# ajzhai/PEANUT

Measured on AMD Instinct MI355X. Metric: maps/sec for 480x480x(4+N_cat) prediction fwd, batch 32, higher is better.
Workload: dtype f32; 1 GPU; 480x480, 14-channel (4+10) partial maps -> 6-class prediction forward (PSPNet R50-V1c-D8), batch 32 per GPU, seeded random-init weights; survey_config=2, global_batch=32, parallelism=dp1 (map shards, no data-path collective)

## Files before the change

include/peanut_hip.h:

```cpp
#ifndef PEANUT_HIP_H_
#define PEANUT_HIP_H_

#include <stddef.h>
#include <stdint.h>

#ifdef __cplusplus
extern "C" {
#endif

#define PEANUT_OK 0
#define PEANUT_EINVAL (-2)
#define PEANUT_EHIP (-3)
#define PEANUT_EWEIGHTS (-4)
#define PEANUT_ERANGE (-5)

const char* peanut_last_error(void);
const char* peanut_last_conv_kernel(void);
int peanut_abi_version(void);
const char* peanut_build_arch(void);
const char* peanut_source_hash(void);
int peanut_debug_weight_pieces(const float* values, int n, int precision, unsigned short* pieces, float* pack_scale);
int peanut_debug_wino_weights(const float* w_oihw, int cout, int cin, int tile, float* out);
long long peanut_debug_deferred_splitk_count(void);
int peanut_debug_lds_canary(int workgroups, int lds_bytes, int rounds, int* mismatches, void* stream);
int peanut_debug_pkfma_canary(int workgroups, int rounds, int* mismatches, void* stream);

int peanut_set_default_option(const char* key, long long value);
int peanut_get_default_option(const char* key, long long* value);
const char* peanut_option_list(void);


typedef struct peanut_pred_cfg {
  int in_channels;
  int num_classes;
  int strides[4];
  int dilations[4];
  int contract_dilation;
  int pool_scales[8];
  int n_pool_scales;
  int head_channels;
  int align_corners;
  float bn_eps;
  int precision;
  int fold_ppm;
  int conv_algo;
} peanut_pred_cfg;

#define PEANUT_ALGO_AUTO 0
#define PEANUT_ALGO_DIRECT 1

#define PEANUT_PREC_FP32 0
#define PEANUT_PREC_BF16X3 1
#define PEANUT_PREC_FP16X3 2
#define PEANUT_PREC_BF16X6 3

typedef struct peanut_tensor {
// ... 191 lines not shown
```

peanut_amd/_lib.py:

```python
from __future__ import annotations

import ctypes as C
import os
import threading

import torch

from . import build as _build

_LOCK = threading.Lock()
_LIB = None
ABI_VERSION = 17


class PeanutHipError(RuntimeError):
    pass


class PeanutRangeError(PeanutHipError, FloatingPointError):
    """PEANUT_ERANGE: precision fp16x3 and a value left fp16's exponent range (include/peanut_hip.h)."""


class PredCfgC(C.Structure):
    _fields_ = [
        ("in_channels", C.c_int), ("num_classes", C.c_int),
        ("strides", C.c_int * 4), ("dilations", C.c_int * 4), ("contract_dilation", C.c_int),
        ("pool_scales", C.c_int * 8), ("n_pool_scales", C.c_int),
        ("head_channels", C.c_int), ("align_corners", C.c_int), ("bn_eps", C.c_float),
        ("precision", C.c_int), ("fold_ppm", C.c_int), ("conv_algo", C.c_int),
    ]


class MapCfgC(C.Structure):
    _fields_ = [
        ("frame_height", C.c_int), ("frame_width", C.c_int), ("map_resolution", C.c_int),
        ("map_size_cm", C.c_int), ("global_downscaling", C.c_int), ("vision_range", C.c_int),
        ("hfov", C.c_double), ("du_scale", C.c_int),
        ("cat_pred_threshold", C.c_double), ("exp_pred_threshold", C.c_double),
        ("map_pred_threshold", C.c_double), ("num_sem_categories", C.c_int), ("camera_height", C.c_double),
    ]


class RcnnCfgC(C.Structure):
    _fields_ = [
        ("depth", C.c_int), ("stem_out", C.c_int), ("res2_out", C.c_int), ("stride_in_1x1", C.c_int),
        ("fpn_out", C.c_int), ("num_anchors", C.c_int), ("min_size", C.c_int), ("max_size", C.c_int),
        ("size_divisibility", C.c_int), ("pixel_mean", C.c_float * 3), ("pixel_std", C.c_float * 3),
        ("bn_eps", C.c_float), ("precision", C.c_int), ("conv_algo", C.c_int),
        ("anchor_sizes", C.c_float * 5), ("aspect_ratios", C.c_float * 8),
        ("rpn_pre_nms_topk", C.c_int), ("rpn_post_nms_topk", C.c_int), ("rpn_nms_thresh", C.c_float),
        ("rpn_bbox_weights", C.c_float * 4), ("num_classes", C.c_int), ("box_pooler_resolution", C.c_int),
        ("mask_pooler_resolution", C.c_int), ("fc_dim", C.c_int), ("mask_conv_dim", C.c_int), ("num_mask_convs", C.c_int),
        ("roi_bbox_weights", C.c_float * 4), ("score_thresh_test", C.c_float), ("nms_thresh_test", C.c_float),
        ("detections_per_image", C.c_int), ("mask_threshold", C.c_float),
    ]


class TensorC(C.Structure):
    _fields_ = [("name", C.c_char_p), ("data", C.c_void_p), ("ndim", C.c_int), ("shape", C.c_int64 * 4)]


_P = C.c_void_p
SIGNATURES = {
    "peanut_last_error": (C.c_char_p, []),
    "peanut_last_conv_kernel": (C.c_char_p, []),
    "peanut_abi_version": (C.c_int, []),
    "peanut_build_arch": (C.c_char_p, []),
    "peanut_source_hash": (C.c_char_p, []),
    "peanut_debug_weight_pieces": (C.c_int, [C.c_void_p, C.c_int, C.c_int, C.c_void_p, C.POINTER(C.c_float)]),
    "peanut_debug_wino_weights": (C.c_int, [C.c_void_p, C.c_int, C.c_int, C.c_int, C.c_void_p]),
    "peanut_debug_deferred_splitk_count": (C.c_longlong, []),
    "peanut_debug_lds_canary": (C.c_int, [C.c_int, C.c_int, C.c_int, C.c_void_p, C.c_void_p]),
    "peanut_debug_pkfma_canary": (C.c_int, [C.c_int, C.c_int, C.c_void_p, C.c_void_p]),
    "peanut_pred_create": (C.c_int, [C.POINTER(_P), C.POINTER(PredCfgC), C.POINTER(TensorC), C.c_int]),
    "peanut_pred_destroy": (None, [_P]),
    "peanut_pred_forward": (C.c_int, [_P, _P, _P, C.c_int, C.c_int, C.c_int, C.c_int, _P]),
    "peanut_pred_workspace_bytes": (C.c_size_t, [_P, C.c_int, C.c_int, C.c_int]),
    "peanut_pred_flops_per_map": (C.c_double, [_P, C.c_int, C.c_int]),
    "peanut_pred_debug_keep": (C.c_int, [_P, C.c_int]),
    "peanut_pred_debug_tensor": (C.c_int, [_P, C.c_char_p, C.POINTER(_P), C.POINTER(C.c_int * 4)]),
    "peanut_pred_debug_read": (C.c_int, [_P, C.c_char_p, _P, C.c_size_t, C.POINTER(C.c_int * 4), _P]),
    "peanut_pred_probe_enable": (C.c_int, [_P, C.c_int]),
    "peanut_pred_use_graph": (C.c_int, [_P, C.c_int]),
    "peanut_map_use_graph": (C.c_int, [_P, C.c_int]),
    "peanut_map_mark_agent": (C.c_int, [_P, C.c_int, C.c_int, C.c_int, C.c_int, C.c_int, C.c_int, _P, C.c_int, C.c_int, _P, _P]),
    "peanut_pred_probe_collect": (C.c_int, [_P, C.c_int, C.POINTER(C.c_char_p), C.POINTER(C.c_char_p),
                                            C.POINTER(C.c_double), C.POINTER(C.c_double), C.POINTER(C.c_double),
                                            C.POINTER(C.c_int)]),
    "peanut_map_create": (C.c_int, [C.POINTER(_P), C.POINTER(MapCfgC)]),
    "peanut_map_destroy": (None, [_P]),
    "peanut_map_dims": (C.c_int, [_P, C.POINTER(C.c_int * 4)]),
    "peanut_map_forward": (C.c_int, [_P, _P, _P, _P, _P, _P, _P, _P]),
    "peanut_map_reserve": (C.c_int, [_P, C.c_int]),
    "peanut_map_forward_batch": (C.c_int, [_P, C.c_int, _P, _P, C.POINTER(_P), _P, _P, C.POINTER(_P), _P]),
    "peanut_map_mark_agent_batch": (C.c_int, [C.c_int, C.POINTER(_P), C.c_int, C.c_int, C.POINTER(C.c_int), _P, C.c_int,
                                              C.POINTER(C.c_int), C.POINTER(C.c_int), _P]),
    "peanut_map_debug_launches": (C.c_int, [_P]),
    "peanut_preprocess_obs_batch": (C.c_int, [_P, _P, _P, C.c_int, C.c_int, C.c_int, C.c_int, C.c_int, C.c_double, C.c_double, _P, _P]),
# ... 161 lines not shown
```

peanut_amd/csrc/common.h:

```cpp
#pragma once
#include <hip/hip_runtime.h>
#include <stdint.h>
#include <string>

namespace peanut {

void set_error(const std::string& msg);
int fail(int code, const std::string& msg);
void note_kernel(const char* family);
const char* noted_kernel();

#define PEANUT_HIP_CHECK(expr)                                                            \
  do {                                                                                    \
    hipError_t _e = (expr);                                                               \
    if (_e != hipSuccess)                                                                 \
      return ::peanut::fail(-3, std::string(#expr) + ": " + hipGetErrorString(_e));       \
  } while (0)

struct ConvDesc {
  int cin;
  int cout;
  int kh, kw, stride, pad, dil;
  int relu;
  int bn_tile;
// ... 60 lines not shown
  };
  return at(y0, x0) * wy * wx + at(y0, x0 + 1) * wy * lx + at(y0 + 1, x0) * ly * wx + at(y0 + 1, x0 + 1) * ly * lx;
}

inline int conv_out_dim(int n, int k, int s, int p, int d) { return (n + 2 * p - d * (k - 1) - 1) / s + 1; }

void conv_pick_tiles(int cin_pad, int cout, int* bn_tile, int* bk, bool pointwise = false);
size_t conv_packed_floats(int cin_pad, int cout, int kh, int kw, int bn_tile);
void pack_conv_weights(const float* w_oihw, int cout, int cin_real, int cin_pad, int kh, int kw,
                       int bn_tile, int bk, float* out);
int launch_conv(const ConvDesc& d, const ConvArgs& a, hipStream_t stream);
bool conv_pw_enabled();
bool conv_pw_uses_256(int cout, long long M, int mt_per_group, int bn_tile, int cin);
int conv_pw_256_min_k();
bool conv_pw_uses_256w(int cout, long long M, int mt_per_group, int bn_tile, int cin, int flush_ktiles);
bool conv_pw_narrow_tiles(int cin, int cout, long long M, int bn_tile, int mt_per_group);
bool conv_pw_uses_256p(int cout, long long M, int mt_per_group, int bn_tile, int cin, int flush_ktiles, long long in_pixels = 0);
struct ConvKParams;
bool gemm_skinny_takes(const ConvKParams& p, int bn_tile, size_t ws_floats);
int launch_gemm_skinny(const ConvKParams& p, float* ws, size_t ws_floats, hipStream_t stream);
bool conv_pw_uses_256wp(int cout, long long M, int stride, int mt_per_group, int bn_tile, int c1, int c2, int flush_ktiles);
bool conv_pw_uses_ares(int cin, int cout, long long M, int stride, bool two_source, int flush_ktiles, int bn_tile);

bool conv_patch_eligible(const ConvDesc& d, const ConvArgs& a);
const char* conv_patch_kernel_name(const ConvDesc& d, bool nchw);
bool conv_patch_nchw_eligible(const ConvDesc& d, int B, int Ho, int Wo, int creal);
int launch_conv_patch_nchw(const ConvDesc& d, const float* x_nchw, int creal, float* y, int B, int H, int W, int Ho, int Wo, hipStream_t stream);

void wino_geometry(int B, int H, int W, int dil, int* th, int* tw, long long* n_tiles, long long* m_pad, int gran = 128, int m = 4);
void wino_transform_weights(const float* w_oihw, int cout, int cin, float* out, int m = 4);
int launch_wino_input(const float* x, float* V, int B, int H, int W, int C, int dil, hipStream_t s, int gran = 128, int m = 4, long long m_pad_total = 0,
                      const DeferredSplit* df = nullptr);
bool wino_input_accepts_deferred(int B, int H, int W, int C, int dil, int gran, int m);
long long wino_deferred_count();
int launch_wino_output(const float* Mb, const float* scale, const float* shift, const float* res, float* y,
                       int B, int H, int W, int C, int dil, int relu, hipStream_t s, int gran = 128, int m = 4, long long m_pad_total = 0);

bool gemm_rs_uses_256(int cout, long long M, int mt_per_group, int bn_tile, int cin);
const char* gemm_rs_kernel_name(int cout, long long M, int mt_per_group, int bn_tile, int cin, int planes);
size_t sx_packed_bytes(int cin_pad, int cout, int bn_tile, int planes);
void pack_weights_sx(const float* w, int cout, int cin_real, int cin_pad, int bn_tile, int planes, float wscale, void* out);
float sx_pack_scale(const float* w, size_t n, int planes);
size_t sx_conv_packed_bytes(int cin_pad, int cout, int kh, int kw, int bn_tile, int planes);
void pack_weights_sx_conv(const float* w_oihw, int cout, int cin_real, int cin_pad, int kh, int kw, int bn_tile, int planes,
                          float wscale, void* out);

int launch_nchw_to_nhwc_pad(const float* x, float* y, int B, int C, int H, int W, int Cpad, hipStream_t s);
int launch_maxpool3x3s2(const float* x, float* y, int B, int H, int W, int C, int Ho, int Wo, hipStream_t s);
int launch_ppm_pool(const float* x, float* out, int B, int H, int W, int C, const int* scales, int nscales,
                    hipStream_t s, int scale_rows = 0);
size_t ppm_pool_scratch_floats(int B, int H, int C, const int* scales, int nscales);
int launch_ppm_pool2(const float* x, float* scratch, float* out, int B, int H, int W, int C, const int* scales,
                     int nscales, hipStream_t s, int scale_rows = 0);
int launch_ppm_upsample_concat(const float* table, float* out, int B, int H, int W, int Cp, const int* scales,
                               int nscales, int align_corners, hipStream_t s);
int launch_ppm_conv_term(const float* Q, float* R, int B, int H, int W, int C, const int* scales, int nscales,
                         int align_corners, hipStream_t s, int scale_rows = 0);
int launch_upsample_logits(const float* lo, float* out, int B, int h, int w, int K, int H, int W,
                           int align_corners, int sigmoid, hipStream_t s);

}
```

peanut_amd/csrc/options.h:

```cpp
#pragma once
#include <stdlib.h>
#include <string.h>

#include <string>

namespace peanut {

enum OptionId {
  OPT_PW_GLDS, OPT_PW256_MINK, OPT_PW256_MINTILES, OPT_PW256_PHASE, OPT_PW256_SKIP_PAD, OPT_PW256W_MINK, OPT_PW256W_MINTILES, OPT_PW256P_MINK, OPT_PW256P_MINTILES, OPT_PW256P_FLUSH, OPT_PW256P_ORDER, OPT_PW256P_STREAMK, OPT_PW256WP_MINK, OPT_PW256WP_MINTILES, OPT_PW256WP_NPRE, OPT_PW256WP_STAGGER, OPT_PW_ARES, OPT_PW_SKINNY,
  OPT_PW_ARES_MINUNITS, OPT_PATCH_MINTILES, OPT_STEM_NCHW, OPT_BN64_MAXK, OPT_PW_BN64_MAXK, OPT_PW64_MAXTILES, OPT_FP32_BK, OPT_NCHUNK, OPT_RES_PREFETCH, OPT_SPLIT_MODEL,
  OPT_RS_CONV, OPT_RS_BN64_MAXK, OPT_RS256_MINK, OPT_RS256_MINTILES, OPT_RS64_MAXK, OPT_RS64_MAXTILES,
  OPT_WINO_M, OPT_WINO_HEAD_M, OPT_WINO6_MAXDIL, OPT_WINO5_MINDIL, OPT_WINO_FLUSH_CH, OPT_WINO_MIN_CIN, OPT_WINO_NARROW_MINPIX, OPT_WINO_SMALL_MAXWG, OPT_DEFER_SPLITK,
  OPT_PPM_OVERLAP, OPT_PPM_GROUPED, OPT_PPM_TERM_ROWS, OPT_PPM_GROUP_ROWS, OPT_RCNN_WINO_M, OPT_RCNN_STEM_S2D, OPT_RCNN_RPN_FUSED, OPT_RCNN_FPN_OVERLAP, OPT_RCNN_RANK_SORT, OPT_RCNN_TOPK_SLICE, OPT_RCNN_NMS_LEVELS, OPT_FMM_LOCAL32, OPT_FMM_MAX_PASSES, OPT_FMM_BLOCKED, OPT_FMM_INNER,
  OPT_COUNT
};

struct OptionInfo {
  const char* key;
  long long def;
  bool upload_time;
  const char* help;
};

inline const OptionInfo* option_table() {
  static const OptionInfo t[OPT_COUNT] = {
      {"pw_glds", 1, false, "fp32 1x1 convs / grouped GEMMs on the LDS-DMA kernels of conv_pw.hip (0: conv_igemm)"},
      {"pw256_mink", 1024, false, "fewest input channels for the 256 x 128 three-stage kernel"},
      {"pw256_mintiles", 256, false, "fewest 256 x 128 tiles for that kernel"},
      {"pw256_phase", 1, false, "the two waves of a SIMD request their LDS-DMA pieces half an iteration apart"},
      {"pw256_skip_pad", 1, false, "256 x 128 kernel, grouped GEMMs: waves whose rows are all group padding issue no MFMAs (0: compute the zero rows)"},
      {"pw256w_mink", 768, false, "fewest input channels for the 256 x 256 two-stage kernel (0: off)"},
      {"pw256w_mintiles", 1536, false, "fewest 256 x 256 tiles for that kernel"},
      {"pw256p_mink", 512, false, "fewest input channels for the persistent 256 x 128 kernel (conv_pw256p.hip; 0: off)"},
      {"pw256p_mintiles", 512, false, "fewest 256 x 128 tiles for that kernel"},
      {"pw256p_flush", 512, false, "most input channels of a Winograd position GEMM (two-level accumulation) that runs on the persistent kernel (0: none)"},
      {"pw256p_order", 1, false, "persistent 256 x 128 kernel: 1 = the workgroups of an XCD walk its run of tiles side by side (neighbours share operand panels in L2), 0 = one contiguous run per workgroup"},
      {"pw256p_streamk", 1, false, "persistent 256 x 128 kernel: the tail tiles' k-tiles as one stream in equal runs per workgroup (0: every tail tile cut into the same number of parts)"},
      {"pw256wp_mink", 512, false, "fewest input channels for the persistent 256 x 256 kernel (conv_pw256wp.hip; 0: off)"},
      {"pw256wp_mintiles", 768, false, "fewest 256 x 256 tiles for that kernel"},
      {"pw256wp_npre", 0, false, "persistent 256 x 256 kernel: accumulator blocks per in-place epilogue group (2 or 4; 0 = two with a residual, four without)"},
      {"pw256wp_stagger", 0, false, "persistent 256 x 256 kernel: spread of the workgroups' start times in sleeps of ~3.4 us (their tile boundaries -- 512 KiB of epilogue traffic per CU -- then fall at different times)"},
      {"pw_ares", 1, false, "K = 128 / 256 pointwise layers on the persistent A-resident kernel (conv_pw_ares.hip)"},
      {"pw_skinny", 1, false, "grouped pointwise launches with at most 64 data rows per group (the PSP pyramid's per-scale convs and Q tables at batch 1) on the skinny weight-streaming kernel (gemm_skinny.hip: 6 KiB of LDS, fits next to any other kernel; 0: the MFMA kernels on 128-row padded tiles)"},
      {"pw_ares_minunits", 512, false, "fewest (m-tile, n-tile) units for that kernel"},
      {"patch_mintiles", 1024, false, "3x3 convs of 16 / 32 input channels on the persistent LDS-patch kernel (conv_patch.hip) from this many 8 x 16 output tiles (0: off)"},
      {"stem_nchw", 1, false, "prediction forward: the first stem conv reads the NCHW input itself (conv_patch.hip, NCHW variant) instead of a layout pass + NHWC conv (fp32 mode, when the patch kernel takes the layer)"},
      {"bn64_maxk", 256, true, "128 x 64 tiles for layers with at most this many input channels"},
      {"pw_bn64_maxk", 128, true, "pointwise layers / Winograd position GEMMs: weights PACKED 64 wide up to this many input channels (wider layers: 128-wide packing, 64-wide tiles chosen per shape)"},
      {"pw64_maxtiles", 512, false, "a 128-wide-packed pointwise layer with at most bn64_maxk input channels runs 128 x 64 tiles while its 128 x 128 tiling has fewer tiles than this (two per CU)"},
      {"fp32_bk", 0, true, "16: force 16-channel k-tiles in conv_igemm (experiment)"},
      {"nchunk", 8, false, "n-tiles per chunk of the tile order (0: n fastest over all n-tiles)"},
      {"res_prefetch", 1, false, "request the first residual rows before the last k-tile's MFMAs"},
      {"split_model", 1, false, "tail split-K plan counts CUs (1) or resident slots (0)"},
      {"rs_conv", 1, true, "emulated modes: non-pointwise convs on conv_rs.hip (0: fp32 MFMA kernel)"},
      {"rs_bn64_maxk", 128, true, "emulated modes: 128 x 64 tiles up to this many input channels"},
      {"rs256_mink", 512, false, "emulated modes: fewest input channels for the 256 x 256 kernel"},
      {"rs256_mintiles", 256, false, "emulated modes: fewest 256 x 256 tiles for it"},
      {"rs64_maxk", 512, false, "emulated modes: 64 x 64 tiles up to this many input channels"},
      {"rs64_maxtiles", 128, false, "emulated modes: ... and below this many 128-row tiles"},
      {"wino_m", 0, true, "4 / 5 / 6: force one Winograd form on every eligible layer (0: policy)"},
      {"wino_head_m", 0, true, "4 / 5 / 6: Winograd form of the PSP bottleneck (0: policy)"},
      {"wino6_maxdil", 4, true, "largest dilation that gets an F(6x6) form"},
      {"wino5_mindil", 4, true, "smallest dilation that also gets an F(5x5) form (0: none)"},
      {"wino_flush_ch", 64, true, "channels per partial sum of the position GEMMs' two-level accumulation (0: off)"},
      {"wino_min_cin", 0, true, "fewest input channels of a Winograd layer (0: the planner's policy)"},
      {"wino_narrow_minpix", 20000, false, "layers under 128 channels take their Winograd form from this many input pixels on (round 6: 100 000 -> 20 000 -- with the small-problem transforms one 720 x 720 map's layer1 conv2, 32 400 pixels, gains 5 us per layer as F(6x6); profiles/r9e)"},
      {"wino_small_maxwg", 1024, false, "Winograd transforms: launches with fewer workgroups than this of the one-thread-per-tile kernels take the small-problem variants (a workgroup per tile and 64-channel slice, a thread per line, through LDS; bit-identical; 0: never)"},
      {"defer_splitk", 1, false, "a Bottleneck conv1 whose every tile is split along k leaves its partial tiles unsummed and conv2's (small-problem) Winograd input transform sums them: one launch fewer per block at batch 1, bit-identical (0: every conv runs its own reduce); read when a (B, H, W) plan is built"},
      {"ppm_overlap", -1, false, "pyramid branch of the PSP head on a side stream: 0 / 1, -1 = by size"},
      {"ppm_grouped", -1, false, "per-scale PSP GEMMs as one grouped launch: 0 / 1, -1 = by size"},
      {"ppm_term_rows", 1, false, "folded pyramid term: one wave per output row, no barrier in the row loop (0: the workgroup-wide two-phase kernel)"},
      {"ppm_group_rows", 0, false, "pyramid pooling, row pass: rows added up per workgroup (1..5; 0 = by size: as many as still leave ~768 workgroups)"},
      {"rcnn_wino_m", 0, true, "detector front end: 4 / 5 / 6 pins one Winograd form (0: per shape)"},
      {"rcnn_stem_s2d", 1, true, "detector stem 7x7 stride 2 as a space-to-depth 4x4 conv"},
      {"rcnn_rpn_fused", 1, false, "detector: the RPN head on all five pyramid levels as one chain (five input transforms, ONE grouped Winograd GEMM, five output transforms, one objectness and one anchor-delta GEMM over all levels' rows: 12 launches instead of 25); read when a (B, H, W) plan is built"},
      {"rcnn_fpn_overlap", 0, false, "detector: the FPN output convs of p5, p4, p3 on a side stream next to the lateral / top-down chain that ends in p2's (round 5 experiment, bit-identical; measured SLOWER at batch 1, 5.70 against 5.61 ms per frame, profiles/r8: off); read when a (B, H, W) plan is built"},
      {"rcnn_rank_sort", 1, false, "detector: the RPN candidates of an image are ordered by counting the larger keys (n / 64 workgroups) instead of one workgroup's bitonic sort (round 5; same order: the keys are distinct)"},
      {"rcnn_topk_slice", 20480, false, "detector: objectness logits per workgroup of the per-level top-k (a level is cut into up to 8 ranges whose k largest are merged by counting; 0: one workgroup per level, round 4)"},
      {"rcnn_nms_levels", 1, false, "detector: the proposal NMS level by level (five 16 x 16-word suppression blocks and five scans per image side by side, post-NMS top-k by counting) instead of one score-sorted list per image (round 5; same proposals)"},
      {"fmm_local32", 1, false, "goal solver: single-precision local solve inside a tile"},
      {"fmm_max_passes", 24, false, "goal solver: hard ceiling of the second-order ordering passes; they stop as soon as a pass changes nothing (6-10 passes on the agent's 960 x 960 map; peanut_goal_converged reports whether they reached their fixed point)"},
      {"fmm_blocked", 1, false, "goal solver: a wave relaxes its 8 x 8 block of the tile to convergence between workgroup barriers (round 5; 0: one Jacobi sweep of the whole tile per barrier pair)"},
      {"fmm_inner", 48, false, "goal solver: iterations a wave spends on its block before it publishes it (blocked rounds)"},
  };
  return t;
}

struct Options {
  long long v[OPT_COUNT];
};

inline int option_index(const char* key) {
  if (!key) return -1;
  std::string k(key);
  for (auto& c : k) c = (char)((c >= 'A' && c <= 'Z') ? c - 'A' + 'a' : c);
  if (k.rfind("peanut_", 0) == 0) k = k.substr(7);
  const OptionInfo* t = option_table();
  for (int i = 0; i < OPT_COUNT; ++i)
    if (k == t[i].key) return i;
  return -1;
// ... 38 lines not shown
```

peanut_amd/csrc/pred_api.hip:

```cpp
#include <math.h>
#include <string.h>

#include <map>
#include <memory>
#include <string>
#include <vector>

#include "net_common.h"

namespace peanut {

static thread_local std::string g_err;
void set_error(const std::string& msg) { g_err = msg; }
int fail(int code, const std::string& msg) {
  g_err = msg;
  return code;
}
static thread_local const char* g_kernel = "";
void note_kernel(const char* family) { g_kernel = family; }
const char* noted_kernel() { return g_kernel; }

namespace {

enum OpKind { OP_TO_NHWC, OP_CONV, OP_CONV_NCHW, OP_MAXPOOL, OP_PPM_POOL, OP_PPM_UP, OP_PPM_TERM, OP_UPSAMPLE, OP_WINO_IN, OP_WINO_GEMM, OP_WINO_OUT };
// ... 174 lines not shown
  }
  if (d.rs == 2) return std::string(d.s_planes == 3 ? "conv_rs6_128x" : (d.s_planes == 4 ? "conv_rs3h_128x" : "conv_rs3_128x")) + std::to_string(d.bn_tile);
  if (d.rs) return gemm_rs_kernel_name(d.cout, M, mt_per_group, d.bn_tile, d.cin, d.s_planes);
  if (d.bk == 32 && d.kh == 1 && d.kw == 1 && d.pad == 0 && (!two_source || d.stride == 1) && d.cin % 32 == 0 && conv_pw_enabled())
  {
    const int flush = d.flush_ch / d.bk;
    if (conv_pw_uses_256wp(d.cout, M, d.stride, mt_per_group, d.bn_tile, d.cin, 0, flush))
      return "conv_pw_glds_256x256p";
    if (conv_pw_uses_ares(d.cin, d.cout, M, d.stride, two_source, flush, d.bn_tile)) return "conv_pw_ares_128x128";
    if (conv_pw_uses_256w(d.cout, M, mt_per_group, d.bn_tile, d.cin, flush)) return "conv_pw_glds_256x256";
    if (conv_pw_uses_256p(d.cout, M, mt_per_group, d.bn_tile, d.cin, flush, M * d.stride * d.stride)) return "conv_pw_glds_256x128p";
    if (conv_pw_uses_256(d.cout, M, mt_per_group, d.bn_tile, d.cin)) return "conv_pw_glds_256x128";
    if (conv_pw_narrow_tiles(d.cin, d.cout, M, d.bn_tile, mt_per_group)) return "conv_pw_glds_128x64";
    return "conv_pw_glds_128x" + std::to_string(d.bn_tile);
  }
  return "conv_igemm_128x" + std::to_string(d.bn_tile) + "x" + std::to_string(d.bk);
}

void push_conv(Plan& pl, const ConvLayer* L, const Act& in, const Act* in2, const Act* res, const Act& out, Arena* ar = nullptr) {
  const bool wino = L->has_wino && !in2 && ar && (long long)in.B * in.H * in.W >= wino_min_pixels(L->d.cin);
  if (wino) L = wino_pick_form(L, in.B, in.H, in.W);
  if (wino) {
    int th, tw;
    long long n_tiles, m_pad;
    const bool rs_gemm = L->wino.rs != 0;
    const int gran = wino_gran_for(*L, in.B, in.H, in.W);
    wino_geometry(in.B, in.H, in.W, L->d.dil, &th, &tw, &n_tiles, &m_pad, gran, L->wino_m);
    const double np = (double)L->wino_np();
    const long long npl = L->wino_np();
    Act v = make_act(*ar, 1, 1, (int)(npl * m_pad), in.C);
    Act m = make_act(*ar, 1, 1, (int)(npl * m_pad), L->d.cout);
    const std::string fam = L->wino_m == 6 ? "wino6_" : (L->wino_m == 5 ? "wino5_" : "wino_");
    const std::string tag = "[" + fam;
    Op a; a.kind = OP_WINO_IN; a.name = L->name + tag + "in]"; a.kernel = fam + "input"; a.conv = L; a.in = in; a.out = v;
    a.wino_gran = gran;
    a.bytes = (double)in.bytes + np * (double)n_tiles * in.C * 4.0;
    pl.ops.push_back(a);
    Op g; g.kind = OP_WINO_GEMM; g.name = L->name + tag + "gemm]"; g.kernel = conv_kernel_name(L->wino, false, npl * m_pad, (int)(m_pad / 128)); g.conv = L;
    g.in = v; g.in.W = (int)(npl * m_pad); g.in.C = in.C; g.out = m; g.wino_mt_per_group = (int)(m_pad / 128); g.wino_gran = gran; g.wino_valid_rows = (int)n_tiles;
    g.flops = 2.0 * np * (double)m_pad * L->d.cout * L->cin_real;
    g.bytes = np * (double)m_pad * (in.C * 4.0 + L->d.cout * 4.0) +
              np * (rs_gemm ? (double)L->wino_group_bytes : (double)L->wino_group_floats * 4);
    pl.ops.push_back(g);
    Op o; o.kind = OP_WINO_OUT; o.name = L->name + tag + "out]"; o.kernel = fam + "output"; o.conv = L; o.in = m; o.out = out;
    if (res) { o.res = *res; o.has_res = true; }
    o.wino_gran = gran;
    o.bytes = np * (double)n_tiles * L->d.cout * 4 + (double)out.bytes + (res ? (double)out.bytes : 0.0);
    pl.ops.push_back(o);
    ar->release(v.off, v.bytes);
    ar->release(m.off, m.bytes);
    return;
  }
  Op op;
  op.kind = OP_CONV; op.name = L->name; op.conv = L; op.in = in; op.out = out;
  op.kernel = conv_kernel_name(L->d, in2 != nullptr, (long long)out.B * out.H * out.W, 0, &out, res != nullptr);
  if (in2) { op.in2 = *in2; op.has_in2 = true; }
  if (res) { op.res = *res; op.has_res = true; }
  op.flops = conv_flops(L, out);
  op.bytes = (double)in.bytes + (in2 ? (double)in2->bytes : 0.0) + (double)out.bytes + (res ? (double)out.bytes : 0.0) +
             (L->d.rs == 2 ? (double)sx_conv_packed_bytes(L->d.cin, L->d.cout, L->d.kh, L->d.kw, L->d.bn_tile, L->d.s_planes)
              : L->d.rs ? (double)sx_packed_bytes(L->d.cin, L->d.cout, L->d.bn_tile, L->d.s_planes)
                      : (double)conv_packed_floats(L->d.cin, L->d.cout, L->d.kh, L->d.kw, L->d.bn_tile) * 4);
  pl.ops.push_back(op);
}

std::unique_ptr<Plan> build_plan(const peanut_pred* h, int B, int H, int W) {
  auto pl = std::make_unique<Plan>();
// ... 281 lines not shown
      a.x = P(op.in); a.y = P(op.out);
      a.B = 1; a.H = 1; a.W = op.in.W; a.c1 = op.in.C; a.c2 = 0; a.Ho = 1; a.Wo = op.in.W;
      a.ws = P(op.branch ? pl.splitk2 : pl.splitk); a.ws_floats = kSplitKScratchFloats;
      a.mt_per_group = op.wino_mt_per_group;
      a.group_valid_rows = op.wino_valid_rows;
      a.w_group_stride = op.conv->wino.rs ? op.conv->wino_group_bytes : op.conv->wino_group_floats;
      return launch_conv(op.conv->wino, a, s);
    }
    case OP_WINO_OUT:
      return launch_wino_output(P(op.in), op.conv->d.scale, op.conv->d.shift, op.has_res ? P(op.res) : nullptr, P(op.out),
                                op.out.B, op.out.H, op.out.W, op.out.C, op.conv->d.dil, op.conv->d.relu, s, op.wino_gran, op.conv->wino_m);
    case OP_MAXPOOL:
      return launch_maxpool3x3s2(P(op.in), P(op.out), op.in.B, op.in.H, op.in.W, op.in.C, op.out.H, op.out.W, s);
    case OP_PPM_POOL:
      return launch_ppm_pool2(P(op.in), op.has_in2 ? P(op.in2) : nullptr, P(op.out), op.in.B, op.in.H, op.in.W, op.in.C,
                              h->cfg.pool_scales, h->cfg.n_pool_scales, s, op.ppm_scale_rows);
    case OP_PPM_UP:
      return launch_ppm_upsample_concat(P(op.in), P(op.out), op.out.B, op.out.H, op.out.W, h->cfg.head_channels,
                                        h->cfg.pool_scales, h->cfg.n_pool_scales, h->cfg.align_corners, s);
    case OP_PPM_TERM:
      return launch_ppm_conv_term(P(op.in), P(op.out), op.out.B, op.out.H, op.out.W, h->cfg.head_channels,
                                  h->cfg.pool_scales, h->cfg.n_pool_scales, h->cfg.align_corners, s, op.ppm_scale_rows);
    case OP_UPSAMPLE:
      return launch_upsample_logits(P(op.in), out_dev, op.in.B, op.in.H, op.in.W, op.in.C, pl.H, pl.W,
                                    h->cfg.align_corners, sigmoid, s);
  }
  return fail(PEANUT_EINVAL, "unknown op");
}

extern "C" {

const char* peanut_last_error(void) { return g_err.c_str(); }
const char* peanut_last_conv_kernel(void) { return noted_kernel(); }
int peanut_abi_version(void) { return 17; }
const char* peanut_build_arch(void) { return "gfx950"; }
#ifndef PEANUT_SOURCE_HASH
#define PEANUT_SOURCE_HASH ""
#endif
const char* peanut_source_hash(void) { return PEANUT_SOURCE_HASH; }

namespace {
int option_lookup(const char* key, const char* who) {
  const int i = option_index(key);
  if (i < 0) return fail(PEANUT_EINVAL, std::string(who) + ": unknown option '" + (key ? key : "(null)") + "'");
  return i;
}
int handle_set_option(Options& o, const char* key, long long value, const char* who) {
  const int i = option_lookup(key, who);
  if (i < 0) return i;
  if (option_table()[i].upload_time)
    return fail(PEANUT_EINVAL, std::string(who) + ": option '" + option_table()[i].key +
                                   "' shapes the uploaded weights; set it with peanut_set_default_option before creating the handle");
  o.v[i] = value;
  return 0;
}
}

int peanut_set_default_option(const char* key, long long value) {
  const int i = option_lookup(key, "peanut_set_default_option");
  if (i < 0) return i;
  default_options().v[i] = value;
  return 0;
}
int peanut_get_default_option(const char* key, long long* value) {
  const int i = option_lookup(key, "peanut_get_default_option");
  if (i < 0) return i;
  if (value) *value = default_options().v[i];
// ... 314 lines not shown
  a.x = x; a.x2 = x2; a.res = res; a.y = y; a.B = B; a.H = H; a.W = W;
  a.c1 = x2 ? c1 : d.cin;
  a.c2 = x2 ? d.cin - c1 : 0;
  a.Ho = conv_out_dim(H, d.kh, d.stride, d.pad, d.dil);
  a.Wo = conv_out_dim(W, d.kw, d.stride, d.pad, d.dil);
  if (a.Ho < 1 || a.Wo < 1) return fail(PEANUT_EINVAL, "peanut_conv_forward: empty output");
  if (int rc = c->ws.ensure(kSplitKScratchFloats * sizeof(float))) return rc;
  a.ws = (float*)c->ws.p; a.ws_floats = kSplitKScratchFloats;
  if (c->L.has_wino && !x2) {
    size_t vf, mf;
    wino_scratch_floats(c->L, B, H, W, &vf, &mf);
    if (vf * sizeof(float) > c->wino_v.bytes || mf * sizeof(float) > c->wino_m.bytes) PEANUT_HIP_CHECK(hipDeviceSynchronize());
    if (int rc = c->wino_v.ensure(vf * sizeof(float))) return rc;
    if (int rc = c->wino_m.ensure(mf * sizeof(float))) return rc;
  }
  return launch_conv_layer(c->L, a, (float*)c->wino_v.p, (float*)c->wino_m.p, (hipStream_t)stream);
}

int peanut_debug_weight_pieces(const float* values, int n, int precision, unsigned short* pieces, float* pack_scale) {
  const int planes = rs_planes_of(precision);
  if (!values || !pieces || !pack_scale || n < 1 || !planes) return fail(PEANUT_EINVAL, "peanut_debug_weight_pieces: bad arguments");
  const int cin_pad = (n + 15) / 16 * 16, bn = 64, np = planes == 4 ? 2 : planes;
  *pack_scale = sx_pack_scale(values, (size_t)n, planes);
  std::vector<unsigned char> packed(sx_packed_bytes(cin_pad, 1, bn, planes));
  pack_weights_sx(values, 1, n, cin_pad, bn, planes, *pack_scale, packed.data());
  const unsigned short* o = reinterpret_cast<const unsigned short*>(packed.data());
  for (int q = 0; q < 3; ++q)
    for (int c = 0; c < n; ++c)
      pieces[(size_t)q * n + c] = q < np ? o[((size_t)(c / 16) * np + q) * bn * 16 + (c % 16)] : (unsigned short)0;
  return 0;
}

long long peanut_debug_deferred_splitk_count(void) { return wino_deferred_count(); }

int peanut_debug_wino_weights(const float* w_oihw, int cout, int cin, int tile, float* out) {
  if (!w_oihw || !out || cout < 1 || cin < 1 || tile < 4 || tile > 6) return fail(PEANUT_EINVAL, "peanut_debug_wino_weights: bad arguments");
  wino_transform_weights(w_oihw, cout, cin, out, tile);
  return 0;
}

}
```

peanut_amd/csrc/winograd.hip:

```cpp
#include <stdlib.h>

#include <atomic>

#include "common.h"
#include "conv_common.h"

namespace peanut {

namespace {

template <typename V>
__device__ __forceinline__ V fmak(V a, float k, V c) { return __builtin_elementwise_fma(a, (V)k, c); }

__device__ __forceinline__ void bt6(const f32x4 d0, const f32x4 d1, const f32x4 d2, const f32x4 d3, const f32x4 d4,
                                    const f32x4 d5, f32x4& t0, f32x4& t1, f32x4& t2, f32x4& t3, f32x4& t4, f32x4& t5) {
#pragma clang fp contract(off)
  const f32x4 a = fmak(d2, -2.25f, d4), b = fmak(d3, 0.75f, -1.6875f * d1);
  const f32x4 c = fmak(d2, -0.5625f, d4), e = fmak(d3, 1.5f, -0.84375f * d1);
  t0 = fmak(d0, 1.265625f, fmak(d2, -2.8125f, d4));
  t1 = a + b;
  t2 = a - b;
  t3 = c + e;
  t4 = c - e;
  t5 = fmak(d1, 1.265625f, fmak(d3, -2.8125f, d5));
// ... 623 lines not shown
  }
  __syncthreads();
  if (a >= 4) return;
  const int c = c0 + a * g.d;
  const size_t img = (size_t)b * g.H * g.W;
  f32x4 rc[4];
  if constexpr (RES) {
#pragma unroll
    for (int k = 0; k < 4; ++k) {
      const int r = r0 + k * g.d;
      const bool ok = c < g.W && r < g.H;
      const size_t off = ok ? (img + (size_t)r * g.W + c) * g.C + ng * 4 : 0;
      rc[k] = *reinterpret_cast<const f32x4*>(res + off);
    }
  }
  const f32x4 sc = *reinterpret_cast<const f32x4*>(scale + ng * 4);
  const f32x4 sh = *reinterpret_cast<const f32x4*>(shift + ng * 4);
  f32x4 o0, o1, o2, o3;
  at6(qs[0][a][l], qs[1][a][l], qs[2][a][l], qs[3][a][l], qs[4][a][l], qs[5][a][l], o0, o1, o2, o3);
  if (c >= g.W) return;
  const f32x4 o[4] = {o0, o1, o2, o3};
#pragma unroll
  for (int k = 0; k < 4; ++k) {
    const int r = r0 + k * g.d;
    if (r >= g.H) continue;
    const size_t off = (img + (size_t)r * g.W + c) * g.C + ng * 4;
    f32x4 v = o[k] * sc + sh;
    if constexpr (RES) v += rc[k];
    if (relu) v = relu_keep_nan(v);
    *reinterpret_cast<f32x4*>(y + off) = v;
  }
}

int wino_small_lanes(long long n_tiles, int C, int m) {
  const long long maxwg = opt(OPT_WINO_SMALL_MAXWG);
  if (maxwg <= 0 || (m != 4 && m != 6)) return 0;
  const long long big_wgs = (n_tiles * (m == 4 ? C / 4 : C / 2) + 255) / 256;
  if (big_wgs >= maxwg) return 0;
  const int per32 = m == 4 ? 128 : 64, per16 = per32 / 2;
  const int lanes = C % per32 == 0 ? 32 : (C % per16 == 0 ? 16 : 0);
  if (!lanes || n_tiles * (C / (lanes * (m == 4 ? 4 : 2))) > 0x7fffffffLL) return 0;
  return lanes;
}

int grid_for(long long total) {
  long long blocks = (total + 255) / 256;
  if (blocks > 256LL * 64) blocks = 256LL * 64;
  if (blocks < 1) blocks = 1;
  return (int)blocks;
}

}

void wino_geometry(int B, int H, int W, int dil, int* th, int* tw, long long* n_tiles, long long* m_pad, int gran, int m) {
  const int hs = (H + dil - 1) / dil, wsub = (W + dil - 1) / dil;
  *th = (hs + m - 1) / m;
  *tw = (wsub + m - 1) / m;
  *n_tiles = (long long)B * dil * dil * *th * *tw;
  *m_pad = (*n_tiles + gran - 1) / gran * gran;
}

void wino_transform_weights(const float* w_oihw, int cout, int cin, float* out, int m) {
  static const double G4[6][3] = {{64.0 / 81, 0, 0},
                                  {-128.0 / 243, -32.0 / 81, -8.0 / 27},
                                  {-128.0 / 243, 32.0 / 81, -8.0 / 27},
                                  {32.0 / 243, 16.0 / 81, 8.0 / 27},
                                  {32.0 / 243, -16.0 / 81, 8.0 / 27},
                                  {0, 0, 1}};
  static const double G6[8][3] = {{-1, 0, 0},
                                  {32.0 / 45, 16.0 / 45, 8.0 / 45},
                                  {32.0 / 45, -16.0 / 45, 8.0 / 45},
                                  {-2.0 / 9, -2.0 / 9, -2.0 / 9},
                                  {-2.0 / 9, 2.0 / 9, -2.0 / 9},
                                  {1.0 / 90, 1.0 / 45, 2.0 / 45},
                                  {1.0 / 90, -1.0 / 45, 2.0 / 45},
// ... 2 lines not shown
                                  {16.0 / 15, 8.0 / 15, 4.0 / 15},
                                  {16.0 / 21, -8.0 / 21, 4.0 / 21},
                                  {-1.0 / 3, -1.0 / 3, -1.0 / 3},
                                  {-1.0 / 6, 1.0 / 6, -1.0 / 6},
                                  {1.0 / 210, 1.0 / 70, 3.0 / 70},
                                  {0, 0, 1}};
  const int n_in = m + 2;
  const double (*G)[3] = m == 6 ? G6 : (m == 5 ? G5 : G4);
  const size_t plane = (size_t)cout * cin;
  for (int n = 0; n < cout; ++n)
    for (int c = 0; c < cin; ++c) {
      const float* g = w_oihw + ((size_t)n * cin + c) * 9;
      double t[8][3];
      for (int i = 0; i < n_in; ++i)
        for (int k = 0; k < 3; ++k) t[i][k] = G[i][0] * g[0 * 3 + k] + G[i][1] * g[1 * 3 + k] + G[i][2] * g[2 * 3 + k];
      for (int i = 0; i < n_in; ++i)
        for (int l = 0; l < n_in; ++l)
          out[(size_t)(i * n_in + l) * plane + (size_t)n * cin + c] =
              (float)(t[i][0] * G[l][0] + t[i][1] * G[l][1] + t[i][2] * G[l][2]);
    }
}

static std::atomic<long long> g_deferred_count{0};
long long wino_deferred_count() { return g_deferred_count.load(std::memory_order_relaxed); }

bool wino_input_accepts_deferred(int B, int H, int W, int C, int dil, int gran, int m) {
  if (C % 4 || m < 4 || m > 6 || C % 128 != 0) return false;
  int th, tw;
  long long n_tiles, m_pad;
  wino_geometry(B, H, W, dil, &th, &tw, &n_tiles, &m_pad, gran, m);
  return wino_small_lanes(n_tiles, C, m) != 0;
}

int launch_wino_input(const float* x, float* V, int B, int H, int W, int C, int dil, hipStream_t s, int gran, int m, long long m_pad_total,
                      const DeferredSplit* df) {
  if (C % 4 || m < 4 || m > 6) return fail(-2, "wino_input: channels must be a multiple of 4, tiles 4x4, 5x5 or 6x6");
  WinoGeom g{B, H, W, C, dil, 0, 0, 0, 0};
  wino_geometry(B, H, W, dil, &g.th, &g.tw, &g.n_tiles, &g.m_pad, gran, m);
  if (m_pad_total > 0) g.m_pad = m_pad_total;
  const long long total = g.n_tiles * (m == 4 ? C / 4 : C / 2);
  const bool defer = df && df->valid;
  DeferredSrc src{};
  if (defer) {
    if (df->cout != C || (long long)df->M != (long long)B * H * W || !wino_small_lanes(g.n_tiles, C, m))
      return fail(-2, "wino_input: deferred split-K partials do not match this transform");
    src = DeferredSrc{df->partial, df->scale, df->shift, df->alpha, df->split_p, df->ntiles, df->relu};
    g_deferred_count.fetch_add(1, std::memory_order_relaxed);
  }
  if (const int lanes = wino_small_lanes(g.n_tiles, C, m)) {
    const unsigned grid = (unsigned)(g.n_tiles * (C / (lanes * (m == 4 ? 4 : 2))));
#define PEANUT_WINO_SMALL_IN(K, L, T)                                                                          \
    do {                                                                                                       \
      if (defer && src.split_p == 4) hipLaunchKernelGGL((K<L, 4>), dim3(grid), dim3(T), 0, s, x, V, g, src);   \
      else if (defer && src.split_p == 2) hipLaunchKernelGGL((K<L, 2>), dim3(grid), dim3(T), 0, s, x, V, g, src); \
      else if (defer) hipLaunchKernelGGL((K<L, 0>), dim3(grid), dim3(T), 0, s, x, V, g, src);                  \
      else hipLaunchKernelGGL((K<L, -1>), dim3(grid), dim3(T), 0, s, x, V, g, src);                            \
    } while (0)
    if (m == 6 && lanes == 32) PEANUT_WINO_SMALL_IN(wino6_input_small_kernel, 32, 256);
    else if (m == 6) PEANUT_WINO_SMALL_IN(wino6_input_small_kernel, 16, 128);
    else if (lanes == 32) PEANUT_WINO_SMALL_IN(wino4_input_small_kernel, 32, 192);
    else PEANUT_WINO_SMALL_IN(wino4_input_small_kernel, 16, 96);
#undef PEANUT_WINO_SMALL_IN
  } else if (m == 6) hipLaunchKernelGGL(wino6_input_kernel, dim3(grid_for(total)), dim3(256), 0, s, x, V, g);
  else if (m == 5) hipLaunchKernelGGL(wino5_input_kernel, dim3(grid_for(total)), dim3(256), 0, s, x, V, g);
  else hipLaunchKernelGGL(wino_input_kernel, dim3(grid_for(total)), dim3(256), 0, s, x, V, g);
  hipError_t e = hipGetLastError();
  if (e != hipSuccess) return fail(-3, std::string("wino_input launch: ") + hipGetErrorString(e));
  return 0;
}

int launch_wino_output(const float* Mb, const float* scale, const float* shift, const float* res, float* y,
                       int B, int H, int W, int C, int dil, int relu, hipStream_t s, int gran, int m, long long m_pad_total) {
  if (C % 4 || m < 4 || m > 6) return fail(-2, "wino_output: channels must be a multiple of 4, tiles 4x4, 5x5 or 6x6");
  WinoGeom g{B, H, W, C, dil, 0, 0, 0, 0};
  wino_geometry(B, H, W, dil, &g.th, &g.tw, &g.n_tiles, &g.m_pad, gran, m);
  if (m_pad_total > 0) g.m_pad = m_pad_total;
  const long long total = g.n_tiles * (m == 4 ? C / 4 : C / 2);
  if (const int lanes = wino_small_lanes(g.n_tiles, C, m)) {
    const unsigned grid = (unsigned)(g.n_tiles * (C / (lanes * (m == 4 ? 4 : 2))));
#define PEANUT_WINO_SMALL_OUT(K, R, L, T) hipLaunchKernelGGL((K<R, L>), dim3(grid), dim3(T), 0, s, Mb, scale, shift, res, y, g, relu)
    if (m == 6 && lanes == 32) { if (res) PEANUT_WINO_SMALL_OUT(wino6_output_small_kernel, true, 32, 256); else PEANUT_WINO_SMALL_OUT(wino6_output_small_kernel, false, 32, 256); }
    else if (m == 6) { if (res) PEANUT_WINO_SMALL_OUT(wino6_output_small_kernel, true, 16, 128); else PEANUT_WINO_SMALL_OUT(wino6_output_small_kernel, false, 16, 128); }
    else if (lanes == 32) { if (res) PEANUT_WINO_SMALL_OUT(wino4_output_small_kernel, true, 32, 192); else PEANUT_WINO_SMALL_OUT(wino4_output_small_kernel, false, 32, 192); }
    else { if (res) PEANUT_WINO_SMALL_OUT(wino4_output_small_kernel, true, 16, 96); else PEANUT_WINO_SMALL_OUT(wino4_output_small_kernel, false, 16, 96); }
#undef PEANUT_WINO_SMALL_OUT
  } else if (m == 6 && res) hipLaunchKernelGGL(wino6_output_kernel<true>, dim3(grid_for(total)), dim3(256), 0, s, Mb, scale, shift, res, y, g, relu);
  else if (m == 6) hipLaunchKernelGGL(wino6_output_kernel<false>, dim3(grid_for(total)), dim3(256), 0, s, Mb, scale, shift, res, y, g, relu);
  else if (m == 5) hipLaunchKernelGGL(wino5_output_kernel, dim3(grid_for(total)), dim3(256), 0, s, Mb, scale, shift, res, y, g, relu);
  else if (res) hipLaunchKernelGGL(wino_output_kernel<true>, dim3(grid_for(total)), dim3(256), 0, s, Mb, scale, shift, res, y, g, relu);
  else hipLaunchKernelGGL(wino_output_kernel<false>, dim3(grid_for(total)), dim3(256), 0, s, Mb, scale, shift, res, y, g, relu);
  hipError_t e = hipGetLastError();
  if (e != hipSuccess) return fail(-3, std::string("wino_output launch: ") + hipGetErrorString(e));
  return 0;
}

// ... 2 lines not shown
```

Measured before the change: 893.7 maps/s.

## Add strip-form Winograd F(6x6) input transform sharing column passes through LDS

Adds a new Winograd F(6x6) input-transform kernel for large launches. Each workgroup handles a run of five consecutive tiles in a tile row and an 8-lane channel slice. The column pass is computed once per shared input column and staged in LDS, then each tile's row pass reads it back, with 16-byte loads and stores throughout. This is meant to remove the redundant loads and column transforms that overlapping tiles repeat in the one-thread-per-tile kernel. The cost is LDS use, a barrier, and idle threads in partial strips.

```diff
diff --git a/include/peanut_hip.h b/include/peanut_hip.h
--- a/include/peanut_hip.h
+++ b/include/peanut_hip.h
@@ -22,6 +22,7 @@
 int peanut_debug_weight_pieces(const float* values, int n, int precision, unsigned short* pieces, float* pack_scale);
 int peanut_debug_wino_weights(const float* w_oihw, int cout, int cin, int tile, float* out);
 long long peanut_debug_deferred_splitk_count(void);
+const char* peanut_debug_wino_input_kernel(void);
 int peanut_debug_lds_canary(int workgroups, int lds_bytes, int rounds, int* mismatches, void* stream);
 int peanut_debug_pkfma_canary(int workgroups, int rounds, int* mismatches, void* stream);
 
diff --git a/peanut_amd/_lib.py b/peanut_amd/_lib.py
--- a/peanut_amd/_lib.py
+++ b/peanut_amd/_lib.py
@@ -10,7 +10,7 @@
 
 _LOCK = threading.Lock()
 _LIB = None
-ABI_VERSION = 17
+ABI_VERSION = 18
 
 
 class PeanutHipError(RuntimeError):
@@ -64,6 +64,7 @@
 SIGNATURES = {
     "peanut_last_error": (C.c_char_p, []),
     "peanut_last_conv_kernel": (C.c_char_p, []),
+    "peanut_debug_wino_input_kernel": (C.c_char_p, []),
     "peanut_abi_version": (C.c_int, []),
     "peanut_build_arch": (C.c_char_p, []),
     "peanut_source_hash": (C.c_char_p, []),
diff --git a/peanut_amd/csrc/common.h b/peanut_amd/csrc/common.h
--- a/peanut_amd/csrc/common.h
+++ b/peanut_amd/csrc/common.h
@@ -116,6 +116,8 @@
 int launch_wino_input(const float* x, float* V, int B, int H, int W, int C, int dil, hipStream_t s, int gran = 128, int m = 4, long long m_pad_total = 0,
                       const DeferredSplit* df = nullptr);
 bool wino_input_accepts_deferred(int B, int H, int W, int C, int dil, int gran, int m);
+const char* wino_input_form(int B, int H, int W, int C, int dil, int gran, int m);
+const char* wino_last_input_form();
 long long wino_deferred_count();
 int launch_wino_output(const float* Mb, const float* scale, const float* shift, const float* res, float* y,
                        int B, int H, int W, int C, int dil, int relu, hipStream_t s, int gran = 128, int m = 4, long long m_pad_total = 0);
diff --git a/peanut_amd/csrc/options.h b/peanut_amd/csrc/options.h
--- a/peanut_amd/csrc/options.h
+++ b/peanut_amd/csrc/options.h
@@ -10,7 +10,7 @@
   OPT_PW_GLDS, OPT_PW256_MINK, OPT_PW256_MINTILES, OPT_PW256_PHASE, OPT_PW256_SKIP_PAD, OPT_PW256W_MINK, OPT_PW256W_MINTILES, OPT_PW256P_MINK, OPT_PW256P_MINTILES, OPT_PW256P_FLUSH, OPT_PW256P_ORDER, OPT_PW256P_STREAMK, OPT_PW256WP_MINK, OPT_PW256WP_MINTILES, OPT_PW256WP_NPRE, OPT_PW256WP_STAGGER, OPT_PW_ARES, OPT_PW_SKINNY,
   OPT_PW_ARES_MINUNITS, OPT_PATCH_MINTILES, OPT_STEM_NCHW, OPT_BN64_MAXK, OPT_PW_BN64_MAXK, OPT_PW64_MAXTILES, OPT_FP32_BK, OPT_NCHUNK, OPT_RES_PREFETCH, OPT_SPLIT_MODEL,
   OPT_RS_CONV, OPT_RS_BN64_MAXK, OPT_RS256_MINK, OPT_RS256_MINTILES, OPT_RS64_MAXK, OPT_RS64_MAXTILES,
-  OPT_WINO_M, OPT_WINO_HEAD_M, OPT_WINO6_MAXDIL, OPT_WINO5_MINDIL, OPT_WINO_FLUSH_CH, OPT_WINO_MIN_CIN, OPT_WINO_NARROW_MINPIX, OPT_WINO_SMALL_MAXWG, OPT_DEFER_SPLITK,
+  OPT_WINO_M, OPT_WINO_HEAD_M, OPT_WINO6_MAXDIL, OPT_WINO5_MINDIL, OPT_WINO_FLUSH_CH, OPT_WINO_MIN_CIN, OPT_WINO_NARROW_MINPIX, OPT_WINO_SMALL_MAXWG, OPT_WINO_STRIP, OPT_DEFER_SPLITK,
   OPT_PPM_OVERLAP, OPT_PPM_GROUPED, OPT_PPM_TERM_ROWS, OPT_PPM_GROUP_ROWS, OPT_RCNN_WINO_M, OPT_RCNN_STEM_S2D, OPT_RCNN_RPN_FUSED, OPT_RCNN_FPN_OVERLAP, OPT_RCNN_RANK_SORT, OPT_RCNN_TOPK_SLICE, OPT_RCNN_NMS_LEVELS, OPT_FMM_LOCAL32, OPT_FMM_MAX_PASSES, OPT_FMM_BLOCKED, OPT_FMM_INNER,
   OPT_COUNT
 };
@@ -66,6 +66,7 @@
       {"wino_min_cin", 0, true, "fewest input channels of a Winograd layer (0: the planner's policy)"},
       {"wino_narrow_minpix", 20000, false, "layers under 128 channels take their Winograd form from this many input pixels on (round 6: 100 000 -> 20 000 -- with the small-problem transforms one 720 x 720 map's layer1 conv2, 32 400 pixels, gains 5 us per layer as F(6x6); profiles/r9e)"},
       {"wino_small_maxwg", 1024, false, "Winograd transforms: launches with fewer workgroups than this of the one-thread-per-tile kernels take the small-problem variants (a workgroup per tile and 64-channel slice, a thread per line, through LDS; bit-identical; 0: never)"},
+      {"wino_strip", 1, false, "Winograd F(6x6) input transforms of launches above wino_small_maxwg: 1 = the strip form (a workgroup per run of consecutive tiles of a tile row and channel slice, column pass once per shared column, through LDS, 16-byte accesses; bit-identical), 0 = one thread per tile and channel pair"},
       {"defer_splitk", 1, false, "a Bottleneck conv1 whose every tile is split along k leaves its partial tiles unsummed and conv2's (small-problem) Winograd input transform sums them: one launch fewer per block at batch 1, bit-identical (0: every conv runs its own reduce); read when a (B, H, W) plan is built"},
       {"ppm_overlap", -1, false, "pyramid branch of the PSP head on a side stream: 0 / 1, -1 = by size"},
       {"ppm_grouped", -1, false, "per-scale PSP GEMMs as one grouped launch: 0 / 1, -1 = by size"},
diff --git a/peanut_amd/csrc/pred_api.hip b/peanut_amd/csrc/pred_api.hip
--- a/peanut_amd/csrc/pred_api.hip
+++ b/peanut_amd/csrc/pred_api.hip
@@ -230,7 +230,7 @@
     Act m = make_act(*ar, 1, 1, (int)(npl * m_pad), L->d.cout);
     const std::string fam = L->wino_m == 6 ? "wino6_" : (L->wino_m == 5 ? "wino5_" : "wino_");
     const std::string tag = "[" + fam;
-    Op a; a.kind = OP_WINO_IN; a.name = L->name + tag + "in]"; a.kernel = fam + "input"; a.conv = L; a.in = in; a.out = v;
+    Op a; a.kind = OP_WINO_IN; a.name = L->name + tag + "in]"; a.kernel = wino_input_form(in.B, in.H, in.W, in.C, L->d.dil, gran, L->wino_m); a.conv = L; a.in = in; a.out = v;
     a.wino_gran = gran;
     a.bytes = (double)in.bytes + np * (double)n_tiles * in.C * 4.0;
     pl.ops.push_back(a);
@@ -578,7 +578,7 @@
 
 const char* peanut_last_error(void) { return g_err.c_str(); }
 const char* peanut_last_conv_kernel(void) { return noted_kernel(); }
-int peanut_abi_version(void) { return 17; }
+int peanut_abi_version(void) { return 18; }
 const char* peanut_build_arch(void) { return "gfx950"; }
 #ifndef PEANUT_SOURCE_HASH
 #define PEANUT_SOURCE_HASH ""
@@ -959,6 +959,7 @@
 }
 
 long long peanut_debug_deferred_splitk_count(void) { return wino_deferred_count(); }
+const char* peanut_debug_wino_input_kernel(void) { return wino_last_input_form(); }
 
 int peanut_debug_wino_weights(const float* w_oihw, int cout, int cin, int tile, float* out) {
   if (!w_oihw || !out || cout < 1 || cin < 1 || tile < 4 || tile > 6) return fail(PEANUT_EINVAL, "peanut_debug_wino_weights: bad arguments");
diff --git a/peanut_amd/csrc/winograd.hip b/peanut_amd/csrc/winograd.hip
--- a/peanut_amd/csrc/winograd.hip
+++ b/peanut_amd/csrc/winograd.hip
@@ -679,6 +679,66 @@
   }
 }
 
+__device__ __forceinline__ void bt8_line4(const f32x4 (&d)[8], f32x4 (&t)[8]) {
+  f32x2 lo[8], hi[8];
+#pragma unroll
+  for (int i = 0; i < 8; ++i) { lo[i] = d[i].xy; hi[i] = d[i].zw; }
+  bt8(lo[0], lo[1], lo[2], lo[3], lo[4], lo[5], lo[6], lo[7], lo[0], lo[1], lo[2], lo[3], lo[4], lo[5], lo[6], lo[7]);
+  bt8(hi[0], hi[1], hi[2], hi[3], hi[4], hi[5], hi[6], hi[7], hi[0], hi[1], hi[2], hi[3], hi[4], hi[5], hi[6], hi[7]);
+#pragma unroll
+  for (int i = 0; i < 8; ++i) t[i] = f32x4{lo[i].x, lo[i].y, hi[i].x, hi[i].y};
+}
+
+constexpr int wino6_strip_threads(int t, int lanes) { return ((8 * t > 6 * t + 2 ? 8 * t : 6 * t + 2) * lanes + 63) / 64 * 64; }
+
+template <int T, int LANES>
+__global__ __launch_bounds__(wino6_strip_threads(T, LANES)) void wino6_input_strip_kernel(const float* __restrict__ x, float* __restrict__ V,
+                                                                                         const WinoGeom g, const int strips_per_row) {
+  constexpr int NC = 6 * T + 2;
+  constexpr int PITCH = NC * LANES + ((LANES == 8 && NC % 2 == 0) ? 8 : 0);
+  static_assert(LANES == 8 || LANES == 16, "row pitch chosen for 8 or 16 lanes");
+  __shared__ f32x4 u[8 * PITCH];
+  const int l = threadIdx.x % LANES, a = threadIdx.x / LANES;
+  const int slices = ((g.C >> 2) + LANES - 1) / LANES;
+  const int cg = (int)(blockIdx.x % slices) * LANES + l;
+  const bool lane_ok = cg < (g.C >> 2);
+  const long long strip = blockIdx.x / slices;
+  const int tx0 = (int)(strip % strips_per_row) * T;
+  const long long tile0 = strip / strips_per_row * g.tw + tx0;
+  const int nt = min(T, g.tw - tx0);
+  int b, oy, ox, ty, tx;
+  decode_tile(g, tile0, b, oy, ox, ty, tx);
+  const int r0 = oy + g.d * (6 * ty - 1), c0 = ox + g.d * (6 * tx - 1);
+  if (a < 6 * nt + 2 && lane_ok) {
+    const float* xb = x + (size_t)b * g.H * g.W * g.C + cg * 4;
+    const int c = c0 + a * g.d;
+    const bool cok = (unsigned)c < (unsigned)g.W;
+    f32x4 p[8];
+#pragma unroll
+    for (int i = 0; i < 8; ++i) {
+      const int r = r0 + i * g.d;
+      f32x4 v = {0.f, 0.f, 0.f, 0.f};
+      if (cok && (unsigned)r < (unsigned)g.H) v = *reinterpret_cast<const f32x4*>(xb + ((size_t)r * g.W + c) * g.C);
+      p[i] = v;
+    }
+    bt8_line4(p, p);
+#pragma unroll
+    for (int i = 0; i < 8; ++i) u[i * PITCH + a * LANES + l] = p[i];
+  }
+  __syncthreads();
+  const int t = a / 8, i = a % 8;
+  if (t < nt && lane_ok) {
+    f32x4 q[8];
+#pragma unroll
+    for (int j = 0; j < 8; ++j) q[j] = u[i * PITCH + (6 * t + j) * LANES + l];
+    bt8_line4(q, q);
+    const size_t pos_stride = (size_t)g.m_pad * g.C;
+    float* o = V + (size_t)(tile0 + t) * g.C + cg * 4 + (size_t)(i * 8) * pos_stride;
+#pragma unroll
+    for (int j = 0; j < 8; ++j) *reinterpret_cast<f32x4*>(o + j * pos_stride) = q[j];
+  }
+}
+
 int wino_small_lanes(long long n_tiles, int C, int m) {
   const long long maxwg = opt(OPT_WINO_SMALL_MAXWG);
   if (maxwg <= 0 || (m != 4 && m != 6)) return 0;
@@ -688,6 +748,14 @@
   const int lanes = C % per32 == 0 ? 32 : (C % per16 == 0 ? 16 : 0);
   if (!lanes || n_tiles * (C / (lanes * (m == 4 ? 4 : 2))) > 0x7fffffffLL) return 0;
   return lanes;
+}
+
+constexpr int kStripTiles = 5, kStripLanes = 8;
+long long wino_strip_grid(const WinoGeom& g, int m, int* strips_per_row) {
+  if (opt(OPT_WINO_STRIP) == 0 || m != 6 || wino_small_lanes(g.n_tiles, g.C, m)) return 0;
+  *strips_per_row = (g.tw + kStripTiles - 1) / kStripTiles;
+  const long long wgs = g.n_tiles / g.tw * *strips_per_row * ((g.C / 4 + kStripLanes - 1) / kStripLanes);
+  return wgs <= 0x7fffffffLL ? wgs : 0;
 }
 
 int grid_for(long long total) {
@@ -756,6 +824,17 @@
   return wino_small_lanes(n_tiles, C, m) != 0;
 }
 
+const char* wino_input_form(int B, int H, int W, int C, int dil, int gran, int m) {
+  if (C % 4 || m < 4 || m > 6) return "";
+  WinoGeom g{B, H, W, C, dil, 0, 0, 0, 0};
+  wino_geometry(B, H, W, dil, &g.th, &g.tw, &g.n_tiles, &g.m_pad, gran, m);
+  int strips_per_row = 0;
+  const bool strip = wino_strip_grid(g, m, &strips_per_row) != 0;
+  return strip ? "wino6_input_strip" : (m == 6 ? "wino6_input" : (m == 5 ? "wino5_input" : "wino_input"));
+}
+static thread_local const char* g_input_form = "";
+const char* wino_last_input_form() { return g_input_form; }
+
 int launch_wino_input(const float* x, float* V, int B, int H, int W, int C, int dil, hipStream_t s, int gran, int m, long long m_pad_total,
                       const DeferredSplit* df) {
   if (C % 4 || m < 4 || m > 6) return fail(-2, "wino_input: channels must be a multiple of 4, tiles 4x4, 5x5 or 6x6");
@@ -771,6 +850,8 @@
     src = DeferredSrc{df->partial, df->scale, df->shift, df->alpha, df->split_p, df->ntiles, df->relu};
     g_deferred_count.fetch_add(1, std::memory_order_relaxed);
   }
+  int strips_per_row = 0;
+  g_input_form = wino_input_form(B, H, W, C, dil, gran, m);
   if (const int lanes = wino_small_lanes(g.n_tiles, C, m)) {
     const unsigned grid = (unsigned)(g.n_tiles * (C / (lanes * (m == 4 ? 4 : 2))));
 #define PEANUT_WINO_SMALL_IN(K, L, T)                                                                          \
@@ -785,6 +866,9 @@
     else if (lanes == 32) PEANUT_WINO_SMALL_IN(wino4_input_small_kernel, 32, 192);
     else PEANUT_WINO_SMALL_IN(wino4_input_small_kernel, 16, 96);
 #undef PEANUT_WINO_SMALL_IN
+  } else if (const long long wgs = wino_strip_grid(g, m, &strips_per_row)) {
+    hipLaunchKernelGGL((wino6_input_strip_kernel<kStripTiles, kStripLanes>), dim3((unsigned)wgs), dim3(wino6_strip_threads(kStripTiles, kStripLanes)), 0, s, x, V, g,
+                       strips_per_row);
   } else if (m == 6) hipLaunchKernelGGL(wino6_input_kernel, dim3(grid_for(total)), dim3(256), 0, s, x, V, g);
   else if (m == 5) hipLaunchKernelGGL(wino5_input_kernel, dim3(grid_for(total)), dim3(256), 0, s, x, V, g);
   else hipLaunchKernelGGL(wino_input_kernel, dim3(grid_for(total)), dim3(256), 0, s, x, V, g);
```

New measurement: 893.6 maps/s, median of 2. No clear change (-0.0%).
